# DallinClark/RealTimeRaytracer

Measured on AMD Instinct MI355X. Metric: Mrays/sec at 1920x1080 1spp (all rays: primary + shadow), higher is better.
Workload: dtype f32

## Files before the change

realtimeraytracer_amd/csrc/kernels/rtr_device.h:

```cpp
#pragma once
#include <hip/hip_runtime.h>
#include <stdint.h>
#include "../../../include/rtr_types.h"
#include "../../../include/rtr_math.h"

namespace rtrdev {

struct DeviceTexture { const uint8_t* pixels; uint32_t width, height, channels, _pad; };

constexpr uint32_t kLightTriRecord = 4;

struct DeviceScene {
    const uint4* nodes;
    const RtrBvhGrid* grid;
    const uint4* nodes4;
    uint32_t numNodes4;
    const float4* tris;
    const RtrVertex* vertices;
    const uint32_t* indices;
    const RtrObjectInfo* objects;
    const RtrAreaLightInfo* lights;
    const float4* lightTris;
    const uint32_t* lightTriFirst;
    const float* xforms;
// ... 376 lines not shown
__device__ __forceinline__ size_t out_index(const RenderArgs& ra, uint32_t px, uint32_t lrow, uint32_t gy) {
    return (size_t)(ra.directRows ? gy : lrow) * ra.width + px;
}

__device__ __forceinline__ rtr_v3 primary_dir(const RenderArgs& ra, uint32_t px, uint32_t py, uint32_t i) {
    const float jx = rtr_random(px + i), jy = rtr_random(px + i * 322u);
    const float offx = ((float)px + jx) - 0.5f, offy = ((float)py + jy) - 0.5f;
    const rtr_v3 pw = rtr_madd(rtr_madd(rtr_ld3(ra.cam.topLeftViewportCorner), rtr_ld3(ra.cam.horizontalViewportDelta), offx),
                               rtr_ld3(ra.cam.verticalViewportDelta), offy);
    return rtr_normalize(rtr_sub(pw, rtr_ld3(ra.cam.position)));
}

struct Accum { rtr_v3 analytic, shadowed, unshadowed, avgNormal, avgPosition; };

struct Surface {
    rtr_v3 hitPoint, hitNormal, viewDir, color, mDiffuse, mSpecular;
    float roughness, metallic, om;
    float4 t1, t2;
};

template <bool SHADE, bool STATS>
__device__ __forceinline__ bool fetch_surface(const DeviceScene& sc, const RenderArgs& ra, const HitRec& h, rtr_v3 rayDir,
                                              bool wantAnalytic, Accum& o, Surface& sf, LocalStats& st) {
    if (h.custom == RTR_MISS) {
        if (SHADE) {
            rtr_v3 sky = rtr_ld3(sc.skyLinear);
            if (sc.hdri.pixels) {
                const rtr_v3 dir = rtr_normalize(rayDir);
                const float hu = rtr_atan2(dir.z, dir.x) / (2.0f * 3.14159265f) + 0.5f;
                float hv = rtr_acos(rtr_clamp(dir.y, -1.0f, 1.0f)) / 3.14159265f;
                hv = 1.0f - hv;
                const float4 tx = sample_tex<STATS>(sc.hdri, hu, hv, st);
                sky = rtr_mk(rtr_to_linear(tx.x), rtr_to_linear(tx.y), rtr_to_linear(tx.z));
            }
            o.analytic = rtr_add(o.analytic, sky); o.unshadowed = rtr_add(o.unshadowed, sky); o.shadowed = rtr_add(o.shadowed, sky);
        }
        return false;
    }
    if (h.custom < sc.numLights) {
        if (SHADE) {
            const rtr_v3 lc = rtr_ld3(sc.lights[h.custom].color);
            o.analytic = rtr_add(o.analytic, lc); o.unshadowed = rtr_add(o.unshadowed, lc); o.shadowed = rtr_add(o.shadowed, lc);
        }
        return false;
    }
    const rtr_v3 camPos = rtr_ld3(ra.cam.position);
    if (STATS) st.hits++;
    const RtrObjectInfo* oi = sc.objects + (h.custom - sc.numLights);
    const uint32_t vOff = oi->vertexOffset, iOff = oi->indexOffset;
    const uint32_t i0 = sc.indices[3u * h.prim + 0u + iOff];
    const uint32_t i1 = sc.indices[3u * h.prim + 1u + iOff];
    const uint32_t i2 = sc.indices[3u * h.prim + 2u + iOff];
    const float4* va = reinterpret_cast<const float4*>(sc.vertices + (i0 + vOff));
    const float4* vb = reinterpret_cast<const float4*>(sc.vertices + (i1 + vOff));
    const float4* vc = reinterpret_cast<const float4*>(sc.vertices + (i2 + vOff));
    const rtr_v3 p0 = f4xyz(va[0]), p1 = f4xyz(vb[0]), p2 = f4xyz(vc[0]);
    const rtr_v3 n0 = f4xyz(va[1]), n1 = f4xyz(vb[1]), n2 = f4xyz(vc[1]);
    const float b0 = 1.0f - h.u - h.v, b1 = h.u, b2 = h.v;
    const rtr_v3 localPos = rtr_madd(rtr_madd(rtr_scale(p0, b0), p1, b1), p2, b2);
    const rtr_v3 hitPoint = rtr_xform_point34(sc.xforms + 12u * h.custom, localPos);
    const rtr_v3 nsum = rtr_madd(rtr_madd(rtr_scale(n0, b0), n1, b1), n2, b2);
    const float* nm = sc.nmats + 12u * h.custom;
    rtr_v3 hitNormal;
    if (rtr_dot(nsum, nsum) > 0.0f) {
        hitNormal = rtr_normalize(rtr_mul33(nm, rtr_normalize(nsum)));
    } else {
        const rtr_v3 g = rtr_cross(rtr_sub(p1, p0), rtr_sub(p2, p0));
        rtr_v3 n = rtr_normalize(rtr_mul33(nm, rtr_normalize(g)));
        if (rtr_dot(n, rayDir) > 0.0f) n = rtr_neg(n);
        hitNormal = n;
    }
    float metallic = oi->metallic;
    float rough = oi->specular;
    rtr_v3 color = rtr_mk(0, 0, 0);
    if (SHADE) {
        rtr_v3 col = rtr_ld3(oi->color);
        if (oi->usesColorMap | oi->usesSpecularMap | oi->usesMetallicMap) {
            const float4 ta = va[2], tb = vb[2], tc = vc[2];
            const float uu = rtr_fma(tc.x, b2, rtr_fma(tb.x, b1, ta.x * b0));
            const float vv = rtr_fma(tc.y, b2, rtr_fma(tb.y, b1, ta.y * b0));
            if (oi->usesColorMap != 0u) { const float4 t = sample_tex<STATS>(sc.textures[oi->colorIndex], uu, vv, st); col = rtr_mk(t.x, t.y, t.z); }
            if (oi->usesSpecularMap != 0u) rough = sample_tex<STATS>(sc.textures[oi->specularIndex], uu, vv, st).x;
            if (oi->usesMetallicMap != 0u) metallic = sample_tex<STATS>(sc.textures[oi->metallicIndex], uu, vv, st).x;
        }
        color = rtr_mk(rtr_to_linear(col.x), rtr_to_linear(col.y), rtr_to_linear(col.z));
    }
    const float roughness = 1.0f - rough;

    const rtr_v3 viewDir = rtr_normalize(rtr_sub(camPos, hitPoint));
    const float om = 1.0f - metallic;
    rtr_v3 mDiffuse = rtr_mk(0, 0, 0), mSpecular = rtr_mk(0, 0, 0);
    float4 t1 = make_float4(1, 0, 0, 1), t2 = make_float4(0, 0, 0, 0);
    if (SHADE) {
        o.avgNormal = rtr_add(o.avgNormal, hitNormal);
        o.avgPosition = rtr_add(o.avgPosition, hitPoint);
        mDiffuse = rtr_scale(color, om);
        mSpecular = rtr_mk(rtr_fma(color.x, metallic, 0.04f * om), rtr_fma(color.y, metallic, 0.04f * om),
                           rtr_fma(color.z, metallic, 0.04f * om));
        if (wantAnalytic) {
            const float dotNV = rtr_clamp(rtr_dot(hitNormal, viewDir), 0.0f, 1.0f);
            const float lu = rtr_fma(roughness, RTR_LUT_SCALE, RTR_LUT_BIAS);
            const float lv = rtr_fma(rtr_sqrt(1.0f - dotNV), RTR_LUT_SCALE, RTR_LUT_BIAS);
            t1 = sample_lut(sc.ltc1, lu, lv);
            t2 = sample_lut(sc.ltc2, lu, lv);
        }
    }
    sf.hitPoint = hitPoint; sf.hitNormal = hitNormal; sf.viewDir = viewDir; sf.color = color;
    sf.mDiffuse = mDiffuse; sf.mSpecular = mSpecular; sf.roughness = roughness; sf.metallic = metallic; sf.om = om;
    sf.t1 = t1; sf.t2 = t2;
    return true;
}

__device__ __forceinline__ rtr_v3 surface_diffuse(float om, rtr_v3 color) {
    return rtr_mk((om * color.x) / RTR_PI_F, (om * color.y) / RTR_PI_F, (om * color.z) / RTR_PI_F);
}
__device__ __forceinline__ rtr_v3 area_sample_contrib(rtr_v3 hitNormal, rtr_v3 viewDir, float roughness, rtr_v3 mSpecular, rtr_v3 currDiffuse,
                                                      rtr_v3 lcol, float lintensity, float pdf, rtr_v3 sampledLightDir, float lightDistance) {
    const rtr_v3 halfVector = rtr_normalize(rtr_add(viewDir, sampledLightDir));
    const float cosTheta = rtr_clamp(rtr_dot(viewDir, halfVector), 0.0f, 1.0f);
    const float Dg = GGX_Distribution(hitNormal, halfVector, roughness);
    const float G = GGX_PartialGeometryTerm(viewDir, hitNormal, halfVector, roughness) *
                    GGX_PartialGeometryTerm(sampledLightDir, hitNormal, halfVector, roughness);
    const rtr_v3 F = Fresnel_Schlick(cosTheta, mSpecular);
    const float NdotV = rtr_max(rtr_dot(hitNormal, viewDir), 0.1f);
    const float NdotL = rtr_max(rtr_dot(hitNormal, sampledLightDir), 0.1f);
    const float den = 4.0f * NdotV * NdotL;
    const rtr_v3 currSpecular = rtr_mk(((Dg * F.x) * G) / den, ((Dg * F.y) * G) / den, ((Dg * F.z) * G) / den);
    const float attenuation = 1.0f / (lightDistance * lightDistance);
    const rtr_v3 BRDF = rtr_add(currSpecular, currDiffuse);
    const rtr_v3 Lr = rtr_mk((((lcol.x * lintensity) * NdotL) * attenuation) * 10.0f, (((lcol.y * lintensity) * NdotL) * attenuation) * 10.0f,
                             (((lcol.z * lintensity) * NdotL) * attenuation) * 10.0f);
    return rtr_mk((BRDF.x * Lr.x) / pdf, (BRDF.y * Lr.y) / pdf, (BRDF.z * Lr.z) / pdf);
}
__device__ __forceinline__ rtr_v3 directional_light_dir() { return rtr_normalize(rtr_mk(-1.0f, 1.0f, -0.5f)); }
__device__ __forceinline__ rtr_v3 directional_contrib(rtr_v3 hitNormal, rtr_v3 viewDir, float roughness, rtr_v3 mSpecular, rtr_v3 currDiffuse) {
    const rtr_v3 directLightDir = directional_light_dir();
    const rtr_v3 directLightColor = rtr_mk(1.0f, 1.0f, 0.5f);
    const float directLightIntensity = 0.2f;
    const rtr_v3 halfVector = rtr_normalize(rtr_add(viewDir, directLightDir));
    const float cosTheta = rtr_clamp(rtr_dot(viewDir, halfVector), 0.0f, 1.0f);
    const float Dg = GGX_Distribution(hitNormal, halfVector, roughness);
    const float G = GGX_PartialGeometryTerm(viewDir, hitNormal, halfVector, roughness) *
                    GGX_PartialGeometryTerm(directLightDir, hitNormal, halfVector, roughness);
    const rtr_v3 F = Fresnel_Schlick(cosTheta, mSpecular);
    const float NdotV = rtr_max(rtr_dot(hitNormal, viewDir), 5.0f);
    const float NdotL = rtr_max(rtr_dot(hitNormal, directLightDir), 0.0001f);
    const float den = 4.0f * NdotV * NdotL;
    const rtr_v3 currSpecular = rtr_mk(((Dg * F.x) * G) / den, ((Dg * F.y) * G) / den, ((Dg * F.z) * G) / den);
    const rtr_v3 BRDF = rtr_add(currSpecular, currDiffuse);
    const rtr_v3 Lr = rtr_mk(((directLightColor.x * directLightIntensity) * NdotL) * 20.0f, ((directLightColor.y * directLightIntensity) * NdotL) * 20.0f,
                             ((directLightColor.z * directLightIntensity) * NdotL) * 20.0f);
    return rtr_mul(BRDF, Lr);
}
__device__ __forceinline__ rtr_v3 light_sample_pos(const rtr_v3* P, uint32_t s, uint32_t px, uint32_t py, uint32_t frame) {
    const uint32_t seed = s + px * 733u + py * 1933u + frame;
    float r1 = rtr_random(seed), r2 = rtr_random(seed + 100u);
    if (r1 + r2 > 1.0f) { r1 = 1.0f - r1; r2 = 1.0f - r2; }
    return rtr_madd(rtr_madd(P[0], rtr_sub(P[1], P[0]), r1), rtr_sub(P[2], P[0]), r2);
}

constexpr uint32_t kDirectionalSlot = 0xffffffffu;
#ifndef RTR_INTO_EXPR
#define RTR_INTO_EXPR (rtr_dot(hitNormal, lightVec) < 0.0f)
#endif
template <class Policy, bool STATS>
__device__ __forceinline__ void light_loops(const DeviceScene& sc, const RenderArgs& ra, uint32_t px, uint32_t py,
                                            const Surface& sf, uint32_t want, Accum& o, Policy& pol, LocalStats& st) {
    const bool wantAnalytic = (want & 1u) != 0u, wantUnshadowed = (want & 2u) != 0u;
    const rtr_v3 hitPoint = sf.hitPoint, hitNormal = sf.hitNormal, viewDir = sf.viewDir, color = sf.color;
    const rtr_v3 mDiffuse = sf.mDiffuse, mSpecular = sf.mSpecular;
    const float roughness = sf.roughness, om = sf.om;
    const float4 t1 = sf.t1, t2 = sf.t2;
    const rtr_v3 shadowOrigin = rtr_madd(hitPoint, hitNormal, 0.01f);
    const rtr_v3 currDiffuse = surface_diffuse(om, color);

    for (uint32_t li = 0; li < ra.info.numAreaLights; ++li) {
        const RtrAreaLightInfo* L = sc.lights + li;
        if (STATS) st.lightFetch++;
        const rtr_v3 lcol = rtr_ld3(L->color);
        const float lintensity = L->intensity;
        const uint32_t lnt = L->numTriangles;
        const bool twoSided = L->isTwoSided != 0u;
        for (uint32_t ti = 0; ti < lnt; ++ti) {
            if (STATS) st.lightTriFetch++;
            const float4* rec = sc.lightTris + (size_t)(sc.lightTriFirst[li] + ti) * kLightTriRecord;
            const float4 r0 = rec[0], r1 = rec[1], r2 = rec[2], r3 = rec[3];
            rtr_v3 P[3];
            P[0] = rtr_mk(r0.x, r0.y, r0.z); P[1] = rtr_mk(r1.x, r1.y, r1.z); P[2] = rtr_mk(r2.x, r2.y, r2.z);
            const float pdf = r1.w;
            const rtr_v3 lightNormal = rtr_mk(r3.x, r3.y, r3.z);
            if (!twoSided) {
                if (rtr_dot(lightNormal, rtr_sub(hitPoint, P[0])) < 0.0f) continue;
            }
            rtr_v3 shadowedSample = rtr_mk(0, 0, 0), unshadowedSample = rtr_mk(0, 0, 0);
            pol.slots_at((sc.lightTriFirst[li] + ti) * ra.numShadowRays);
            for (uint32_t s = 0; s < ra.numShadowRays; ++s) {
                const rtr_v3 lightSamplePos = light_sample_pos(P, s, px, py, ra.info.frame);
                const rtr_v3 lightVec = rtr_sub(lightSamplePos, hitPoint);
                const rtr_v3 sampledLightDir = rtr_normalize(lightVec);
                const float lightDistance = rtr_length(lightVec);
                const bool occ = pol.occluded(shadowOrigin, sampledLightDir, lightDistance - 0.5f, lightVec, RTR_INTO_EXPR);
                if (Policy::kShade && (wantUnshadowed || !occ)) {
                    const float currShadow = occ ? 0.0f : 1.0f;
                    const rtr_v3 contrib = area_sample_contrib(hitNormal, viewDir, roughness, mSpecular, currDiffuse, lcol, lintensity, pdf, sampledLightDir, lightDistance);
                    shadowedSample = rtr_madd(shadowedSample, contrib, currShadow);
                    unshadowedSample = rtr_add(unshadowedSample, contrib);
                }
            }
            if (Policy::kShade) {
                const float ns = (float)ra.numShadowRays;
                shadowedSample = rtr_mk(shadowedSample.x / ns, shadowedSample.y / ns, shadowedSample.z / ns);
                unshadowedSample = rtr_mk(unshadowedSample.x / ns, unshadowedSample.y / ns, unshadowedSample.z / ns);
                if (wantAnalytic) {
                    const float diffuse = LTC_Evaluate(hitNormal, viewDir, hitPoint, true, t1, P, lightNormal, twoSided, sc.ltc2);
                    const float spec = LTC_Evaluate(hitNormal, viewDir, hitPoint, false, t1, P, lightNormal, twoSided, sc.ltc2);
                    const rtr_v3 fres = rtr_mk(rtr_fma(1.0f - mSpecular.x, t2.y, mSpecular.x * t2.x),
                                               rtr_fma(1.0f - mSpecular.y, t2.y, mSpecular.y * t2.x),
                                               rtr_fma(1.0f - mSpecular.z, t2.y, mSpecular.z * t2.x));
                    o.analytic = rtr_add(o.analytic, rtr_mk(((lcol.x * lintensity) * rtr_fma(mDiffuse.x, diffuse, spec * fres.x)) * 5.0f,
                                                            ((lcol.y * lintensity) * rtr_fma(mDiffuse.y, diffuse, spec * fres.y)) * 5.0f,
                                                            ((lcol.z * lintensity) * rtr_fma(mDiffuse.z, diffuse, spec * fres.z)) * 5.0f));
                }
                o.shadowed = rtr_add(o.shadowed, shadowedSample);
                o.unshadowed = rtr_add(o.unshadowed, unshadowedSample);
            }
        }
    }
    const rtr_v3 directLightDir = directional_light_dir();
    if (rtr_dot(hitNormal, directLightDir) <= 0.0f) return;
    pol.slots_at(kDirectionalSlot);
    const bool occ = pol.occluded(shadowOrigin, directLightDir, 10000.0f, directLightDir, false);
    if (Policy::kShade && (wantUnshadowed || wantAnalytic || !occ)) {
        const float currShadow = occ ? 0.0f : 1.0f;
        const rtr_v3 contrib = directional_contrib(hitNormal, viewDir, roughness, mSpecular, currDiffuse);
        o.shadowed = rtr_madd(o.shadowed, contrib, currShadow);
        o.unshadowed = rtr_add(o.unshadowed, contrib);
        o.analytic = rtr_add(o.analytic, contrib);
    }
}

__device__ __forceinline__ void light_tri_record(const RtrAreaLightInfo* L, const RtrVertex* vertices, const uint32_t* indices,
                                                 uint32_t ti, float4* rec) {
    const uint32_t lvOff = L->vertexOffset, liOff = L->indexOffset;
    const uint32_t j0 = indices[ti * 3u + 0u + liOff];
    const uint32_t j1 = indices[ti * 3u + 1u + liOff];
    const uint32_t j2 = indices[ti * 3u + 2u + liOff];
    rtr_v3 P[3];
    P[0] = rtr_xform_point44cm(L->transform, rtr_ld3(vertices[j0 + lvOff].position));
    P[1] = rtr_xform_point44cm(L->transform, rtr_ld3(vertices[j1 + lvOff].position));
    P[2] = rtr_xform_point44cm(L->transform, rtr_ld3(vertices[j2 + lvOff].position));
    rtr_v3 lightNormal = rtr_cross(rtr_sub(P[2], P[1]), rtr_sub(P[0], P[1]));
    const float area = rtr_length(lightNormal) * 0.5f;
    const float pdf = 1.0f / (area * 0.7f);
    lightNormal = rtr_normalize(lightNormal);
    rec[0] = make_float4(P[0].x, P[0].y, P[0].z, area);
    rec[1] = make_float4(P[1].x, P[1].y, P[1].z, pdf);
    rec[2] = make_float4(P[2].x, P[2].y, P[2].z, 0.f);
    rec[3] = make_float4(lightNormal.x, lightNormal.y, lightNormal.z, 0.f);
}

template <class Policy, bool STATS>
__device__ __forceinline__ void shade_sample(const DeviceScene& sc, const RenderArgs& ra, uint32_t px, uint32_t py,
                                             const HitRec& h, rtr_v3 rayDir, uint32_t want, Accum& o,
                                             Policy& pol, LocalStats& st) {
    Surface sf;
    if (!fetch_surface<Policy::kShade, STATS>(sc, ra, h, rayDir, (want & 1u) != 0u, o, sf, st)) return;
    light_loops<Policy, STATS>(sc, ra, px, py, sf, want, o, pol, st);
}

__device__ __forceinline__ uint32_t tonemap_pack(rtr_v3 c) {
    return rtr_pack_bgra8(rtr_to_srgb(rtr_aces(c.x)), rtr_to_srgb(rtr_aces(c.y)), rtr_to_srgb(rtr_aces(c.z)));
}

struct FrameOut {
    uint32_t* img[8];
    float4* hdr;
};

constexpr uint32_t kMaxBatch = 32;
struct FrameBatch {
    RenderArgs ra[kMaxBatch];
    FrameOut   fo[kMaxBatch];
    uint32_t   n;
};
static_assert(sizeof(FrameBatch) + sizeof(DeviceScene) + 256 <= 16384, "a launch passes DeviceScene + FrameBatch + a few pointers by value");
__device__ __forceinline__ uint32_t batch_frame(uint32_t g, uint32_t planeStride, uint32_t& q) {
    const uint32_t b = (uint32_t)__builtin_amdgcn_readfirstlane((int)(g / planeStride));
    q = g - b * planeStride;
    return b;
}

__device__ __forceinline__ void write_pixel(const RenderArgs& ra, const FrameOut& fo, size_t p, Accum o) {
    const float n = (float)ra.spp;
    rtr_v3 sh = rtr_mk(o.shadowed.x / n, o.shadowed.y / n, o.shadowed.z / n);
    const rtr_v3 un = rtr_mk(o.unshadowed.x / n, o.unshadowed.y / n, o.unshadowed.z / n);
    const rtr_v3 an = rtr_mk(o.analytic.x / n, o.analytic.y / n, o.analytic.z / n);
    if (fo.hdr) {
        if (ra.accumulate) {
            float4 h = fo.hdr[p];
            h.x += sh.x; h.y += sh.y; h.z += sh.z; h.w += 1.0f;
            fo.hdr[p] = h;
            const float inv = (float)(ra.accumulatedFrames + 1u);
            sh = rtr_mk(h.x / inv, h.y / inv, h.z / inv);
        } else {
            fo.hdr[p] = make_float4(sh.x, sh.y, sh.z, 1.0f);
        }
    }
    if (fo.img[1]) fo.img[1][p] = tonemap_pack(sh);
    if (fo.img[2]) fo.img[2][p] = tonemap_pack(un);
    if (fo.img[0]) fo.img[0][p] = tonemap_pack(an);
    if (fo.img[6]) {
        const rtr_v3 a = rtr_normalize(rtr_mk(o.avgNormal.x / n, o.avgNormal.y / n, o.avgNormal.z / n));
        fo.img[6][p] = rtr_pack_bgra8(a.x, a.y, a.z);
    }
    if (fo.img[7]) fo.img[7][p] = rtr_pack_bgra8(o.avgPosition.x / n, o.avgPosition.y / n, o.avgPosition.z / n);
}

__device__ __forceinline__ void write_pixel_framebuffer(const RenderArgs& ra, const FrameOut& fo, size_t p, rtr_v3 shadowed) {
    const float n = (float)ra.spp;
    rtr_v3 sh = rtr_mk(shadowed.x / n, shadowed.y / n, shadowed.z / n);
    if (fo.hdr) {
        if (ra.accumulate) {
            float4 h = fo.hdr[p];
            h.x += sh.x; h.y += sh.y; h.z += sh.z; h.w += 1.0f;
            fo.hdr[p] = h;
            const float inv = (float)(ra.accumulatedFrames + 1u);
            sh = rtr_mk(h.x / inv, h.y / inv, h.z / inv);
        } else {
            fo.hdr[p] = make_float4(sh.x, sh.y, sh.z, 1.0f);
        }
    }
    if (fo.img[1]) fo.img[1][p] = tonemap_pack(sh);
}

}
```

realtimeraytracer_amd/csrc/kernels/rtr_kernels.hip:

```cpp
#include "rtr_kernels.h"

#include <algorithm>
#include <cstdlib>
#include <cstring>

namespace rtrdev {

constexpr int kBlock = 256;

template <bool STATS, int STACK>
struct InlinePolicy {
    static constexpr bool kShade = true;
    __device__ __forceinline__ void slots_at(uint32_t) {}
    const DeviceScene& sc; int32_t* stack; LocalStats& st;
    __device__ __forceinline__ bool occluded(rtr_v3 o, rtr_v3 d, float tmax, rtr_v3, bool) {
        HitRec h;
        return trace<true, STATS, kBlock>(sc, stack, o, d, 0.001f, tmax, h, st);
    }
};

__device__ __forceinline__ uint32_t wave_sum_u32(uint32_t v) {
#pragma unroll
    for (int o = 32; o > 0; o >>= 1) v += __shfl_xor(v, o);
    return v;
// ... 163 lines not shown
    HitRec h;
    if (STATS) trace<false, true, kPrimBlock, 16, 8>(sc, stack, camPos, dir, 0.001f, 10000.0f, h, st);
    else {
        const uint32_t oct = ray_octant(sc, camPos, dir);
        const uint32_t woct = (uint32_t)__builtin_amdgcn_readfirstlane((int)oct);
        switch (__ballot(oct != woct) != 0ull ? 8u : woct) {
            case 0: trace<false, false, kPrimBlock, 16, 0>(sc, stack, camPos, dir, 0.001f, 10000.0f, h, st); break;
            case 1: trace<false, false, kPrimBlock, 16, 1>(sc, stack, camPos, dir, 0.001f, 10000.0f, h, st); break;
            case 2: trace<false, false, kPrimBlock, 16, 2>(sc, stack, camPos, dir, 0.001f, 10000.0f, h, st); break;
            case 3: trace<false, false, kPrimBlock, 16, 3>(sc, stack, camPos, dir, 0.001f, 10000.0f, h, st); break;
            case 4: trace<false, false, kPrimBlock, 16, 4>(sc, stack, camPos, dir, 0.001f, 10000.0f, h, st); break;
            case 5: trace<false, false, kPrimBlock, 16, 5>(sc, stack, camPos, dir, 0.001f, 10000.0f, h, st); break;
            case 6: trace<false, false, kPrimBlock, 16, 6>(sc, stack, camPos, dir, 0.001f, 10000.0f, h, st); break;
            case 7: trace<false, false, kPrimBlock, 16, 7>(sc, stack, camPos, dir, 0.001f, 10000.0f, h, st); break;
            default: trace<false, false, kPrimBlock, 16, 8>(sc, stack, camPos, dir, 0.001f, 10000.0f, h, st); break;
        }
    }
    const size_t k = (size_t)plane * planeBlocks * kPrimBlock + q;
    if (h.custom == RTR_STACK_OVERFLOW) redoList[atomicAdd(redoCount, 1u)] = (uint32_t)k;
    else {
        hitTuvp[k] = make_float4(h.t, h.u, h.v, __uint_as_float(h.prim));
        hitCustom[k] = h.custom;
        origin_leaf_store(rayOrigin, k, h.leaf);
    }
    if (STATS) st.flush(stats);
}

template <bool STATS>
__global__ __launch_bounds__(kBlock) void k_primary_packet(DeviceScene sc, FrameBatch fb, float4* hitTuvp, uint32_t* hitCustom, float4* rayOrigin, Counters* stats, uint32_t planeBlocks) {
    __shared__ uint4 s_stack[kBlock / 64][64];
    const uint32_t wave = threadIdx.x >> 6, lane = threadIdx.x & 63u;
    const uint32_t plane = blockIdx.x / planeBlocks;
    const RenderArgs& ra = fb.ra[plane / fb.ra[0].spp];
    const uint32_t i = plane % fb.ra[0].spp;
    const uint32_t q = (blockIdx.x - plane * planeBlocks) * kBlock + threadIdx.x;
    uint32_t px = 0, lrow = 0, py = 0;
    const bool valid = pixel_of(ra, q, px, lrow, py);
    unsigned long long active = __ballot(valid);
    if (active == 0ull) return;
    LocalStats st;
    const rtr_v3 o = rtr_ld3(ra.cam.position);
    const rtr_v3 d = valid ? primary_dir(ra, px, py, i) : rtr_mk(0.f, 0.f, 1.f);
    const float tmin = 0.001f, tmax = 10000.0f;
    if (STATS && valid) { st.rays++; st.primary++; }
    const rtr_v3 idir = rtr_mk(rtr_safe_rcp_dir(d.x), rtr_safe_rcp_dir(d.y), rtr_safe_rcp_dir(d.z));
    rtr_v3 ga, gb;
    rtr_ray_grid(o, idir, sc.grid->origin, sc.grid->scale, &ga, &gb);
    HitRec best; best.t = tmax; best.u = 0.f; best.v = 0.f; best.custom = RTR_MISS; best.prim = RTR_MISS; best.leaf = 0;
    const uint4* __restrict__ nodes = sc.nodes;
    const float4* __restrict__ tris = sc.tris;
    uint32_t sp = 0;
    int32_t cur = 0;
    for (;;) {
        const bool mine = ((active >> lane) & 1ull) != 0ull;
        bool pop = true;
        if (cur >= 0) {
            const uint4 a = nodes[2 * cur], b = nodes[2 * cur + 1];
            if (STATS && mine) st.nodes++;
            float tl = 0.f, tr = 0.f;
            const bool hl = mine && slab_pair(a.x, a.y, b.x, ga, gb, tmin, best.t, tl);
            const bool hr = mine && slab_pair(a.z, a.w, b.y, ga, gb, tmin, best.t, tr);
            const unsigned long long mL = __ballot(hl), mR = __ballot(hr);
            if ((mL | mR) != 0ull) {
                pop = false;
                if (mR == 0ull) { cur = (int32_t)b.z; active = mL; }
                else if (mL == 0ull) { cur = (int32_t)b.w; active = mR; }
                else {
                    const uint32_t rNear = (uint32_t)__popcll(__ballot(hl && hr && tr < tl)), lNear = (uint32_t)__popcll(__ballot(hl && hr && !(tr < tl)));
                    const bool rFirst = rNear > lNear;
                    if (lane == 0u) {
                        const unsigned long long m2 = rFirst ? mL : mR;
                        s_stack[wave][sp] = make_uint4(rFirst ? b.z : b.w, (uint32_t)m2, (uint32_t)(m2 >> 32), 0u);
                    }
                    ++sp;
                    cur = (int32_t)(rFirst ? b.w : b.z); active = rFirst ? mR : mL;
                }
            }
        } else {
            const uint32_t code = (uint32_t)~cur;
            const uint32_t first = code >> 3, cnt = (code & 7u) + 1u;
            for (uint32_t k = 0; k < cnt; ++k) {
                const float4 q0 = tris[3u * (first + k)], q1 = tris[3u * (first + k) + 1u], q2 = tris[3u * (first + k) + 2u];
                if (mine) {
                    if (STATS) st.tris++;
                    float t, u, v;
                    if (rtr_mt_intersect(o, d, f4xyz(q0), f4xyz(q1), f4xyz(q2), tmin, &t, &u, &v) && t < tmax) {
                        const uint32_t cu = __float_as_uint(q0.w), pr = __float_as_uint(q1.w);
                        if (!(__float_as_uint(q2.w) & 1u) || alpha_pass<STATS>(sc, cu, pr, u, v, st)) {
                            if (t < best.t || (t == best.t && (cu < best.custom || (cu == best.custom && pr < best.prim)))) {
                                best.t = t; best.u = u; best.v = v; best.custom = cu; best.prim = pr; best.leaf = cur;
                            }
                        }
                    }
                }
            }
        }
        if (pop) {
            if (sp == 0u) break;
            --sp;
            const uint4 e = s_stack[wave][sp];
            cur = __builtin_amdgcn_readfirstlane((int32_t)e.x);
            active = (unsigned long long)(uint32_t)__builtin_amdgcn_readfirstlane((int)e.y) | ((unsigned long long)(uint32_t)__builtin_amdgcn_readfirstlane((int)e.z) << 32);
        }
    }
    if (valid) {
        const size_t k = (size_t)plane * planeBlocks * kBlock + q;
        hitTuvp[k] = make_float4(best.t, best.u, best.v, __uint_as_float(best.prim));
        hitCustom[k] = best.custom;
        origin_leaf_store(rayOrigin, k, best.leaf);
    }
    if (STATS) st.flush(stats);
}

template <bool STATS>
__global__ __launch_bounds__(kBlock) void k_primary_tail(DeviceScene sc, FrameBatch fb, float4* hitTuvp, uint32_t* hitCustom, float4* rayOrigin,
                                                         const uint32_t* __restrict__ redoCount, const uint32_t* __restrict__ redoList,
                                                         int32_t* __restrict__ spill, uint32_t planeStride, Counters* stats) {
    const uint32_t n = *redoCount;
    if (n == 0) return;
    int32_t* stack = spill + blockIdx.x * kBlock + threadIdx.x;
    LocalStats st;
    for (uint32_t j = blockIdx.x * kBlock + threadIdx.x; j < n; j += gridDim.x * kBlock) {
        const uint32_t k = redoList[j];
        const uint32_t plane = k / planeStride, q = k % planeStride;
        const RenderArgs& ra = fb.ra[plane / fb.ra[0].spp];
        const uint32_t i = plane % fb.ra[0].spp;
        uint32_t px, lrow, py;
        if (!pixel_of(ra, q, px, lrow, py)) continue;
        HitRec h;
        trace<false, STATS, 64 * kBlock>(sc, stack, rtr_ld3(ra.cam.position), primary_dir(ra, px, py, i), 0.001f, 10000.0f, h, st);
        if (STATS) { st.rays--; st.primary--; }
        hitTuvp[k] = make_float4(h.t, h.u, h.v, __uint_as_float(h.prim));
        hitCustom[k] = h.custom;
        origin_leaf_store(rayOrigin, k, h.leaf);
    }
    if (STATS) st.flush(stats);
}

__device__ __forceinline__ uint32_t wave_sum(uint32_t v) {
#pragma unroll
    for (int o = 32; o > 0; o >>= 1) v += __shfl_xor(v, o);
    return v;
}
__device__ __forceinline__ uint32_t wave_total(uint32_t v) {
    v += (uint32_t)__builtin_amdgcn_update_dpp(0, (int)v, 0xB1, 0xf, 0xf, false);
    v += (uint32_t)__builtin_amdgcn_update_dpp(0, (int)v, 0x4E, 0xf, 0xf, false);
    v += (uint32_t)__builtin_amdgcn_update_dpp(0, (int)v, 0x141, 0xf, 0xf, false);
    v += (uint32_t)__builtin_amdgcn_update_dpp(0, (int)v, 0x140, 0xf, 0xf, false);
    v += (uint32_t)__builtin_amdgcn_update_dpp(0, (int)v, 0x142, 0xa, 0xf, false);
    v += (uint32_t)__builtin_amdgcn_update_dpp(0, (int)v, 0x143, 0xc, 0xf, false);
    return (uint32_t)__builtin_amdgcn_readlane((int)v, 63);
}

constexpr uint32_t kGenBlock = 1024;
__global__ __launch_bounds__(kGenBlock) void k_shadow_gen(DeviceScene sc, FrameBatch fb, const float4* hitTuvp,
                                                          const uint32_t* hitCustom, RayQueue queue, uint32_t* count, uint32_t planeStride) {
    __shared__ uint32_t s_off[kGenBlock / 64], s_tot[kGenBlock / 64], s_base;
    uint32_t q;
    const uint32_t frame = batch_frame(blockIdx.x * kGenBlock + threadIdx.x, planeStride, q);
    const RenderArgs& ra = fb.ra[frame < fb.n ? frame : 0u];
    const size_t plane0 = (size_t)frame * ra.spp;
    const uint32_t wave = threadIdx.x >> 6;
    uint32_t px = 0, lrow = 0, py = 0;
    const bool live = frame < fb.n && pixel_of(ra, q, px, lrow, py);
    LocalStats st;
    Accum acc = zero_accum();
    const bool single = ra.spp == 1u;
    Surface sf0;
    bool surf0 = false;
    uint32_t n = 0;
    if (live) {
        CountPolicy cp{0};
        for (uint32_t i = 0; i < ra.spp; ++i) {
            const size_t k = (plane0 + i) * planeStride + q;
            const float4 r = hitTuvp[k];
            HitRec h; h.t = r.x; h.u = r.y; h.v = r.z; h.prim = __float_as_uint(r.w); h.custom = hitCustom[k];
            Surface sf;
            const bool surf = fetch_surface<false, false>(sc, ra, h, primary_dir(ra, px, py, i), false, acc, sf, st);
            if (surf) light_loops<CountPolicy, false>(sc, ra, px, py, sf, 0u, acc, cp, st);
            if (i == 0) { sf0 = sf; surf0 = surf; }
        }
        n = cp.n;
    }
    const uint32_t total = wave_sum(n);
    if ((threadIdx.x & 63u) == 0) { s_tot[wave] = total; s_off[wave] = 0; }
    __syncthreads();
    if (threadIdx.x == 0) {
        uint32_t t = 0;
        for (uint32_t w = 0; w < kGenBlock / 64; ++w) t += s_tot[w];
        s_base = t ? atomicAdd(count, t) : 0u;
    }
    __syncthreads();
    uint32_t base = s_base;
    for (uint32_t w = 0; w < wave; ++w) base += s_tot[w];
    if (!live || n == 0) return;
    for (uint32_t i = 0; i < ra.spp; ++i) {
        const size_t k = (plane0 + i) * planeStride + q;
        EmitPolicy pol{queue, (EmitPolicy::lds_word)&s_off[wave], base, (uint32_t)k};
        if (single) {
            if (surf0) { queue_store_origin(queue, k, sf0.hitPoint, sf0.hitNormal); light_loops<EmitPolicy, false>(sc, ra, px, py, sf0, 0u, acc, pol, st); }
        } else {
            const float4 r = hitTuvp[k];
            HitRec h; h.t = r.x; h.u = r.y; h.v = r.z; h.prim = __float_as_uint(r.w); h.custom = hitCustom[k];
            Surface sf;
            if (fetch_surface<false, false>(sc, ra, h, primary_dir(ra, px, py, i), false, acc, sf, st)) {
                queue_store_origin(queue, k, sf.hitPoint, sf.hitNormal);
                light_loops<EmitPolicy, false>(sc, ra, px, py, sf, 0u, acc, pol, st);
            }
        }
    }
}

constexpr size_t kBinnedMinRays = (size_t)10 << 20;
constexpr uint32_t kBinnedMinNodes = 1u << 16;
#ifndef RTR_GEN_OCT_BLOCK
#define RTR_GEN_OCT_BLOCK 512
#endif
constexpr uint32_t kGenOctBlock = RTR_GEN_OCT_BLOCK;
#ifndef RTR_GEN_OCT_WAVES
#define RTR_GEN_OCT_WAVES 7
#endif
#if RTR_GEN_OCT_WAVES > 0
#define RTR_GEN_OCT_ATTR __attribute__((amdgpu_waves_per_eu(RTR_GEN_OCT_WAVES, 8)))
#else
#define RTR_GEN_OCT_ATTR
#endif
__global__ __launch_bounds__(kGenOctBlock) RTR_GEN_OCT_ATTR void k_shadow_gen_oct(DeviceScene sc, FrameBatch fb, const float4* hitTuvp, const uint32_t* hitCustom,
                                                              RayQueue queue, uint32_t* ctrl, uint32_t planeStride, uint2* lists,
                                                              uint32_t listStride, uint32_t kBatch, uint32_t nt) {
    constexpr uint32_t kWaves = kGenOctBlock / 64;
    __shared__ uint32_t s_tot[kWaves][8], s_run[kWaves][8];
    uint32_t q;
    const uint32_t frame = batch_frame(blockIdx.x * kGenOctBlock + threadIdx.x, planeStride, q);
    const RenderArgs& ra = fb.ra[frame < fb.n ? frame : 0u];
    const size_t plane0 = (size_t)frame * ra.spp;
    const uint32_t wave = threadIdx.x >> 6;
    uint32_t px = 0, lrow = 0, py = 0;
    const bool live = frame < fb.n && pixel_of(ra, q, px, lrow, py);
    LocalStats st;
    Accum acc = zero_accum();
    const bool single = ra.spp == 1u;
    Surface sf0;
    bool surf0 = false;
    CountOctPolicy cp{0ull, 0ull};
    if (live) {
        for (uint32_t i = 0; i < ra.spp; ++i) {
            const size_t k = (plane0 + i) * planeStride + q;
            const float4 r = hitTuvp[k];
            HitRec h; h.t = r.x; h.u = r.y; h.v = r.z; h.prim = __float_as_uint(r.w); h.custom = hitCustom[k];
            Surface sf;
            bool surf = fetch_surface<false, false>(sc, ra, h, primary_dir(ra, px, py, i), false, acc, sf, st);
#if RTR_EXP_DOUBLE_FETCH_GEN
            if (surf) {
                HitRec h2 = h; h2.u = h.u + sf.hitPoint.x * (float)(ra.spp - 1u) * 1.0e-30f; h2.v = h.v + sf.hitNormal.y * (float)(ra.spp - 1u) * 1.0e-30f;
                h2.prim = h.prim + (__float_as_uint(sf.hitPoint.z) == 0x7fc12345u ? 1u : 0u);
                Surface sf2;
                if (fetch_surface<false, false>(sc, ra, h2, primary_dir(ra, px, py, i), false, acc, sf2, st)) sf = sf2;
            }
#endif
            if (surf) light_loops<CountOctPolicy, false>(sc, ra, px, py, sf, 0u, acc, cp, st);
            if (i == 0) { sf0 = sf; surf0 = surf; }
        }
    }
    uint32_t mine = 0;
#pragma unroll
    for (uint32_t o = 0; o < 8; ++o) {
        const uint32_t c = (uint32_t)(((o < 4 ? cp.lo : cp.hi) >> ((o & 3u) * 16u)) & 0xffffull);
        mine += c;
        const uint32_t t = wave_total(c);
        if ((threadIdx.x & 63u) == 0) s_tot[wave][o] = t;
    }
    __syncthreads();
    if (threadIdx.x < kQueueLists) {
        const uint32_t o = threadIdx.x / kQueueRegions, x = threadIdx.x % kQueueRegions;
        uint32_t before = 0, len = 0, total = 0;
#pragma unroll
        for (uint32_t oo = 0; oo < 8; ++oo) {
            uint32_t t = 0;
#pragma unroll
            for (uint32_t w = 0; w < kWaves; ++w) t += s_tot[w][oo];
            before += oo < o ? t : 0u;
            len = oo == o ? t : len;
            total += t;
        }
        const uint32_t kB = (kBatch >= 512u && blockIdx.x * 8u >= gridDim.x * 7u) ? kBatch / 2u : kBatch;
        const uint32_t nb = (len + kB - 1) / kB;
        const uint32_t b0 = (x + kQueueRegions - blockIdx.x % kQueueRegions) % kQueueRegions;
        const uint32_t cnt = b0 < nb ? (nb - b0 + kQueueRegions - 1) / kQueueRegions : 0u;
        uint32_t at = 0, pos = 0;
        if (threadIdx.x == 0 && total) at = atomicAdd(ctrl, total);
        if (cnt) pos = atomicAdd(ctrl + kQueueListLens + threadIdx.x, cnt);
        const uint32_t first = (uint32_t)__builtin_amdgcn_readfirstlane((int)at) + before;
        if (x == 0) {
            uint32_t c = first;
            for (uint32_t w = 0; w < kWaves; ++w) { s_run[w][o] = c; c += s_tot[w][o]; }
        }
        for (uint32_t j = 0; j < cnt; ++j) {
            const uint32_t f = (b0 + j * kQueueRegions) * kB;
            lists[(size_t)threadIdx.x * listStride + pos + j] = make_uint2(first + f, len - f < kB ? len - f : kB);
        }
    }
    __syncthreads();
    if (!live || mine == 0) return;
    for (uint32_t i = 0; i < ra.spp; ++i) {
        const size_t k = (plane0 + i) * planeStride + q;
        EmitOctPolicy pol{queue, (EmitOctPolicy::lds_word)&s_run[wave][0], (uint32_t)k, nt};
        if (single) {
            if (surf0) { queue_store_origin(queue, k, sf0.hitPoint, sf0.hitNormal); light_loops<EmitOctPolicy, false>(sc, ra, px, py, sf0, 0u, acc, pol, st); }
        } else {
            const float4 r = hitTuvp[k];
            HitRec h; h.t = r.x; h.u = r.y; h.v = r.z; h.prim = __float_as_uint(r.w); h.custom = hitCustom[k];
            Surface sf;
            if (fetch_surface<false, false>(sc, ra, h, primary_dir(ra, px, py, i), false, acc, sf, st)) {
                queue_store_origin(queue, k, sf.hitPoint, sf.hitNormal);
                light_loops<EmitOctPolicy, false>(sc, ra, px, py, sf, 0u, acc, pol, st);
            }
        }
    }
}

#ifndef RTR_REFILL_LDS
#define RTR_REFILL_LDS 1
#endif
#ifndef RTR_LIST_SHARE
#define RTR_LIST_SHARE 1
#endif
constexpr int kTailBlocks = 64;
constexpr int32_t kDone = (int32_t)0x80000000;
constexpr int32_t kAbandoned = (int32_t)0x80000001;
constexpr uint32_t kBatchDefault = 256, kBatchLong = 512;
constexpr size_t kBatchLongQueue = (size_t)100 << 20;

constexpr uint32_t kResNone = 3u;
#ifndef RTR_TRACE_BLOCK
#define RTR_TRACE_BLOCK 256
#endif
constexpr int kTraceBlock = RTR_TRACE_BLOCK;
#ifndef RTR_TRI_AUX
#define RTR_TRI_AUX 0
#endif
#ifndef RTR_NODE_AUX
#define RTR_NODE_AUX 0
#endif
#ifndef RTR_SHADOW_STACK
#define RTR_SHADOW_STACK RTR_WIDE_STACK
#endif
#ifndef RTR_TRACE_TOP
#define RTR_TRACE_TOP 40
#endif
constexpr uint32_t kTopNodes = (uint32_t)RTR_TRACE_TOP * (RTR_TRACE_BLOCK / 256);

template <int STACK>
__global__ __launch_bounds__(kBlock) void k_shadow_trace(DeviceScene sc, const RayQueue queue,
                                                              const uint32_t* __restrict__ count, uint32_t* nextBatch,
                                                              uint8_t* __restrict__ vis, uint32_t visFill, uint32_t kBatch, uint32_t kRefill,
                                                              uint32_t kInnerMin, uint32_t* overflow, uint32_t overflowCap) {
    __shared__ int32_t s_stack[(STACK + 1) * kBlock];
    int32_t* lds = s_stack + threadIdx.x;
    lds[0] = kDone;
    const uint32_t n = *count;
    uint32_t batchPos = 0, batchEnd = 0;
    bool exhausted = false;
    const uint32_t regionLen = ((n + kQueueRegions - 1) / kQueueRegions + kBatch - 1) / kBatch * kBatch;
    const uint32_t myRegion = blockIdx.x % kQueueRegions;
    uint32_t regionTry = 0;
    int32_t cur = kDone;
    int sp = 0;
    rtr_v3 o = rtr_mk(0, 0, 0), d = rtr_mk(0, 0, 0), ga = rtr_mk(0, 0, 0), gb = rtr_mk(0, 0, 0);
    float tmax = 0.f;
    uint32_t slot = 0, rayIndex = 0, res = kResNone, occ = 0;
    const float tmin = 0.001f;
    typedef uint32_t u32x4 __attribute__((ext_vector_type(4)));
    const __amdgpu_buffer_rsrc_t nodeBuf = __builtin_amdgcn_make_buffer_rsrc((void*)sc.nodes, 0, 0xffffffff, 0x00020000);
    const __amdgpu_buffer_rsrc_t triBuf = __builtin_amdgcn_make_buffer_rsrc((void*)sc.tris, 0, 0xffffffff, 0x00020000);

    for (;;) {
        const unsigned long long idle = __ballot(cur == kDone);
        const uint32_t nIdle = (uint32_t)__popcll(idle);
        if (nIdle >= kRefill || nIdle == 64u) {
            if (cur == kDone && res != kResNone) {
                if (res == 2u) { const uint32_t at = atomicAdd(overflow, 1u); if (at < overflowCap) overflow[1u + at] = rayIndex; }
                else { if (res != visFill) vis[slot] = (uint8_t)res; occ += res; }
                res = kResNone;
            }
            if (!exhausted) {
                if (batchPos == batchEnd) {
                    for (;;) {
                        if (regionTry >= kQueueRegions) { exhausted = true; break; }
                        const uint32_t r = (myRegion + regionTry) % kQueueRegions;
                        const uint32_t lo = r * regionLen;
                        uint32_t hi = lo + regionLen; if (hi > n) hi = n;
                        uint32_t b = hi;
                        if (lo < hi) {
                            uint32_t got = 0;
                            if ((threadIdx.x & 63u) == 0) got = atomicAdd(nextBatch + 16u * r, kBatch);
                            got = (uint32_t)__builtin_amdgcn_readfirstlane((int)got);
                            b = got < regionLen ? lo + got : hi;
                        }
                        if (b < hi) { batchPos = b; batchEnd = (b + kBatch < hi) ? b + kBatch : hi; break; }
                        ++regionTry;
                    }
                }
                if (!exhausted) {
                    const uint32_t avail = batchEnd - batchPos;
                    const uint32_t prefix = __builtin_amdgcn_mbcnt_hi((uint32_t)(idle >> 32), __builtin_amdgcn_mbcnt_lo((uint32_t)idle, 0u));
                    if (cur == kDone && prefix < avail) {
                        rayIndex = batchPos + prefix;
                        queue_load(queue, rayIndex, o, d, tmax, slot, 0u);
                        if (!(tmax > tmin)) {
                            if (visFill != 0u) vis[slot] = 0;
                        } else {
                            const rtr_v3 idir = rtr_mk(rtr_safe_rcp_dir(d.x), rtr_safe_rcp_dir(d.y), rtr_safe_rcp_dir(d.z));
                            rtr_ray_grid(o, idir, sc.grid->origin, sc.grid->scale, &ga, &gb);
                            cur = 0; sp = 0; res = 0u;
                        }
                    }
                    batchPos += (nIdle < avail) ? nIdle : avail;
                }
            }
        }
        if (__ballot(cur != kDone) == 0ull) {
            if (exhausted) break;
            continue;
        }
        for (;;) {
            const unsigned long long innerMask = __ballot(cur >= 0);
            if (innerMask == 0ull) break;
            if ((uint32_t)__popcll(innerMask) <= kInnerMin && __ballot(cur < 0 && cur != kDone) != 0ull) break;
            if (cur >= 0) {
                const int32_t nodeOff = cur << 5;
                const u32x4 a = __builtin_amdgcn_raw_buffer_load_b128(nodeBuf, nodeOff, 0, 0);
                const u32x4 b = __builtin_amdgcn_raw_buffer_load_b128(nodeBuf, nodeOff + 16, 0, 0);
                const int32_t top = lds[sp * kBlock];
                float tl, tr;
                const bool hl = slab_pair(a.x, a.y, b.x, ga, gb, tmin, tmax, tl);
                const bool hr = slab_pair(a.z, a.w, b.y, ga, gb, tmin, tmax, tr);
                const bool swap = tr < tl;
                const int32_t c0 = (int32_t)b.z, c1 = (int32_t)b.w;
                const bool both = hl && hr, none = !(hl || hr);
                const bool second = both ? swap : !hl;
                int32_t next = second ? c1 : c0;
                const bool push = both && sp < STACK;
                if (push) { ++sp; lds[sp * kBlock] = swap ? c0 : c1; }
                if (both && !push) { res = 2u; next = kDone; }
                if (none) { next = top; --sp; }
                cur = next;
            }
        }
        if (cur < 0 && cur != kDone) {
            const uint32_t code = (uint32_t)~cur;
            const uint32_t first = code >> 3, cnt = (code & 7u) + 1u;
            bool hit = false;
            for (uint32_t i = 0; i < cnt && !hit; ++i) {
                const int32_t triOff = (int32_t)((first + i) * 48u);
                const u32x4 r0 = __builtin_amdgcn_raw_buffer_load_b128(triBuf, triOff, 0, 0);
                const u32x4 r1 = __builtin_amdgcn_raw_buffer_load_b128(triBuf, triOff + 16, 0, 0);
                const u32x4 r2 = __builtin_amdgcn_raw_buffer_load_b128(triBuf, triOff + 32, 0, 0);
                const float4 q0 = make_float4(__uint_as_float(r0.x), __uint_as_float(r0.y), __uint_as_float(r0.z), __uint_as_float(r0.w));
                const float4 q1 = make_float4(__uint_as_float(r1.x), __uint_as_float(r1.y), __uint_as_float(r1.z), __uint_as_float(r1.w));
                const float4 q2 = make_float4(__uint_as_float(r2.x), __uint_as_float(r2.y), __uint_as_float(r2.z), __uint_as_float(r2.w));
                float t, u, v;
                if (rtr_mt_intersect(o, d, f4xyz(q0), f4xyz(q1), f4xyz(q2), tmin, &t, &u, &v) && t < tmax) {
                    hit = true;
                    if (__float_as_uint(q2.w) & 1u) {
                        LocalStats st;
                        hit = alpha_pass<false>(sc, __float_as_uint(q0.w), __float_as_uint(q1.w), u, v, st);
                    }
                }
// ... 1112 lines not shown
```

Before: 16490.

## Park shadow sample pairs and hit surface in LDS across count/emit passes

Shadow-ray generation kernels now precompute each pixel's light-sample random pairs once into LDS columns when the shadow-ray count is small, reusing them in both the counting and emitting passes. The octant generator also parks the single-spp hit point and normal in LDS instead of keeping a full Surface live in registers across the block barrier, and reduces per-wave totals in grouped register batches. The intent is to cut recomputation of RNG and lower register pressure so more waves fit. In exchange it uses a large LDS allocation per block, which may itself limit occupancy, and it drops the live/surface check before the emit loop, relying on mine==0 for pixels with no hit.

```diff
diff --git a/realtimeraytracer_amd/csrc/kernels/rtr_device.h b/realtimeraytracer_amd/csrc/kernels/rtr_device.h
--- a/realtimeraytracer_amd/csrc/kernels/rtr_device.h
+++ b/realtimeraytracer_amd/csrc/kernels/rtr_device.h
@@ -552,20 +552,31 @@
                              ((directLightColor.z * directLightIntensity) * NdotL) * 20.0f);
     return rtr_mul(BRDF, Lr);
 }
-__device__ __forceinline__ rtr_v3 light_sample_pos(const rtr_v3* P, uint32_t s, uint32_t px, uint32_t py, uint32_t frame) {
-    const uint32_t seed = s + px * 733u + py * 1933u + frame;
+struct SamplePair { float r1, r2; };
+__device__ __forceinline__ uint32_t light_sample_seed0(uint32_t px, uint32_t py, uint32_t frame) { return px * 733u + py * 1933u + frame; }
+__device__ __forceinline__ SamplePair light_sample_pair(uint32_t seed) {
     float r1 = rtr_random(seed), r2 = rtr_random(seed + 100u);
     if (r1 + r2 > 1.0f) { r1 = 1.0f - r1; r2 = 1.0f - r2; }
-    return rtr_madd(rtr_madd(P[0], rtr_sub(P[1], P[0]), r1), rtr_sub(P[2], P[0]), r2);
-}
+    return SamplePair{r1, r2};
+}
+__device__ __forceinline__ rtr_v3 light_sample_at(const rtr_v3* P, SamplePair r) {
+    return rtr_madd(rtr_madd(P[0], rtr_sub(P[1], P[0]), r.r1), rtr_sub(P[2], P[0]), r.r2);
+}
+__device__ __forceinline__ rtr_v3 light_sample_pos(const rtr_v3* P, uint32_t s, uint32_t px, uint32_t py, uint32_t frame) {
+    return light_sample_at(P, light_sample_pair(s + light_sample_seed0(px, py, frame)));
+}
+struct DrawnSamples {
+    uint32_t px, py, frame;
+    __device__ __forceinline__ SamplePair pair(uint32_t s) const { return light_sample_pair(s + light_sample_seed0(px, py, frame)); }
+};
 
 constexpr uint32_t kDirectionalSlot = 0xffffffffu;
 #ifndef RTR_INTO_EXPR
 #define RTR_INTO_EXPR (rtr_dot(hitNormal, lightVec) < 0.0f)
 #endif
-template <class Policy, bool STATS>
-__device__ __forceinline__ void light_loops(const DeviceScene& sc, const RenderArgs& ra, uint32_t px, uint32_t py,
-                                            const Surface& sf, uint32_t want, Accum& o, Policy& pol, LocalStats& st) {
+template <class Policy, bool STATS, class Samples>
+__device__ __forceinline__ void light_loops_from(const DeviceScene& sc, const RenderArgs& ra, const Samples& smp,
+                                                 const Surface& sf, uint32_t want, Accum& o, Policy& pol, LocalStats& st) {
     const bool wantAnalytic = (want & 1u) != 0u, wantUnshadowed = (want & 2u) != 0u;
     const rtr_v3 hitPoint = sf.hitPoint, hitNormal = sf.hitNormal, viewDir = sf.viewDir, color = sf.color;
     const rtr_v3 mDiffuse = sf.mDiffuse, mSpecular = sf.mSpecular;
@@ -595,7 +606,7 @@
             rtr_v3 shadowedSample = rtr_mk(0, 0, 0), unshadowedSample = rtr_mk(0, 0, 0);
             pol.slots_at((sc.lightTriFirst[li] + ti) * ra.numShadowRays);
             for (uint32_t s = 0; s < ra.numShadowRays; ++s) {
-                const rtr_v3 lightSamplePos = light_sample_pos(P, s, px, py, ra.info.frame);
+                const rtr_v3 lightSamplePos = light_sample_at(P, smp.pair(s));
                 const rtr_v3 lightVec = rtr_sub(lightSamplePos, hitPoint);
                 const rtr_v3 sampledLightDir = rtr_normalize(lightVec);
                 const float lightDistance = rtr_length(lightVec);
@@ -638,6 +649,11 @@
         o.analytic = rtr_add(o.analytic, contrib);
     }
 }
+template <class Policy, bool STATS>
+__device__ __forceinline__ void light_loops(const DeviceScene& sc, const RenderArgs& ra, uint32_t px, uint32_t py,
+                                            const Surface& sf, uint32_t want, Accum& o, Policy& pol, LocalStats& st) {
+    light_loops_from<Policy, STATS>(sc, ra, DrawnSamples{px, py, ra.info.frame}, sf, want, o, pol, st);
+}
 
 __device__ __forceinline__ void light_tri_record(const RtrAreaLightInfo* L, const RtrVertex* vertices, const uint32_t* indices,
                                                  uint32_t ti, float4* rec) {
diff --git a/realtimeraytracer_amd/csrc/kernels/rtr_kernels.hip b/realtimeraytracer_amd/csrc/kernels/rtr_kernels.hip
--- a/realtimeraytracer_amd/csrc/kernels/rtr_kernels.hip
+++ b/realtimeraytracer_amd/csrc/kernels/rtr_kernels.hip
@@ -339,10 +339,31 @@
     return (uint32_t)__builtin_amdgcn_readlane((int)v, 63);
 }
 
+constexpr uint32_t kParkedPairs = 4;
+typedef __attribute__((address_space(3))) uint32_t* lds_column;
+template <uint32_t BLOCK>
+struct ParkedSamples {
+    lds_column pairs;
+    uint32_t seed0;
+    bool parked;
+    __device__ __forceinline__ void draw(uint32_t ns) const {
+        if (!parked) return;
+        for (uint32_t s = 0; s < ns; ++s) {
+            const SamplePair r = light_sample_pair(s + seed0);
+            pairs[2u * s * BLOCK] = __float_as_uint(r.r1); pairs[(2u * s + 1u) * BLOCK] = __float_as_uint(r.r2);
+        }
+    }
+    __device__ __forceinline__ SamplePair pair(uint32_t s) const {
+        if (parked) return SamplePair{__uint_as_float(pairs[2u * s * BLOCK]), __uint_as_float(pairs[(2u * s + 1u) * BLOCK])};
+        return light_sample_pair(s + seed0);
+    }
+};
+
 constexpr uint32_t kGenBlock = 1024;
 __global__ __launch_bounds__(kGenBlock) void k_shadow_gen(DeviceScene sc, FrameBatch fb, const float4* hitTuvp,
                                                           const uint32_t* hitCustom, RayQueue queue, uint32_t* count, uint32_t planeStride) {
     __shared__ uint32_t s_off[kGenBlock / 64], s_tot[kGenBlock / 64], s_base;
+    __shared__ uint32_t s_pairs[2u * kParkedPairs * kGenBlock];
     uint32_t q;
     const uint32_t frame = batch_frame(blockIdx.x * kGenBlock + threadIdx.x, planeStride, q);
     const RenderArgs& ra = fb.ra[frame < fb.n ? frame : 0u];
@@ -356,15 +377,17 @@
     Surface sf0;
     bool surf0 = false;
     uint32_t n = 0;
+    const ParkedSamples<kGenBlock> smp{(lds_column)&s_pairs[threadIdx.x], light_sample_seed0(px, py, ra.info.frame), ra.numShadowRays <= kParkedPairs};
     if (live) {
         CountPolicy cp{0};
+        smp.draw(ra.numShadowRays);
         for (uint32_t i = 0; i < ra.spp; ++i) {
             const size_t k = (plane0 + i) * planeStride + q;
             const float4 r = hitTuvp[k];
             HitRec h; h.t = r.x; h.u = r.y; h.v = r.z; h.prim = __float_as_uint(r.w); h.custom = hitCustom[k];
             Surface sf;
             const bool surf = fetch_surface<false, false>(sc, ra, h, primary_dir(ra, px, py, i), false, acc, sf, st);
-            if (surf) light_loops<CountPolicy, false>(sc, ra, px, py, sf, 0u, acc, cp, st);
+            if (surf) light_loops_from<CountPolicy, false>(sc, ra, smp, sf, 0u, acc, cp, st);
             if (i == 0) { sf0 = sf; surf0 = surf; }
         }
         n = cp.n;
@@ -385,14 +408,14 @@
         const size_t k = (plane0 + i) * planeStride + q;
         EmitPolicy pol{queue, (EmitPolicy::lds_word)&s_off[wave], base, (uint32_t)k};
         if (single) {
-            if (surf0) { queue_store_origin(queue, k, sf0.hitPoint, sf0.hitNormal); light_loops<EmitPolicy, false>(sc, ra, px, py, sf0, 0u, acc, pol, st); }
+            if (surf0) { queue_store_origin(queue, k, sf0.hitPoint, sf0.hitNormal); light_loops_from<EmitPolicy, false>(sc, ra, smp, sf0, 0u, acc, pol, st); }
         } else {
             const float4 r = hitTuvp[k];
             HitRec h; h.t = r.x; h.u = r.y; h.v = r.z; h.prim = __float_as_uint(r.w); h.custom = hitCustom[k];
             Surface sf;
             if (fetch_surface<false, false>(sc, ra, h, primary_dir(ra, px, py, i), false, acc, sf, st)) {
                 queue_store_origin(queue, k, sf.hitPoint, sf.hitNormal);
-                light_loops<EmitPolicy, false>(sc, ra, px, py, sf, 0u, acc, pol, st);
+                light_loops_from<EmitPolicy, false>(sc, ra, smp, sf, 0u, acc, pol, st);
             }
         }
     }
@@ -404,6 +427,7 @@
 #define RTR_GEN_OCT_BLOCK 512
 #endif
 constexpr uint32_t kGenOctBlock = RTR_GEN_OCT_BLOCK;
+constexpr uint32_t kParkSurface = 6, kParkWords = kParkSurface + 2u * kParkedPairs;
 #ifndef RTR_GEN_OCT_WAVES
 #define RTR_GEN_OCT_WAVES 7
 #endif
@@ -417,6 +441,7 @@
                                                               uint32_t listStride, uint32_t kBatch, uint32_t nt) {
     constexpr uint32_t kWaves = kGenOctBlock / 64;
     __shared__ uint32_t s_tot[kWaves][8], s_run[kWaves][8];
+    __shared__ uint32_t s_park[kParkWords * kGenOctBlock];
     uint32_t q;
     const uint32_t frame = batch_frame(blockIdx.x * kGenOctBlock + threadIdx.x, planeStride, q);
     const RenderArgs& ra = fb.ra[frame < fb.n ? frame : 0u];
@@ -427,10 +452,11 @@
     LocalStats st;
     Accum acc = zero_accum();
     const bool single = ra.spp == 1u;
-    Surface sf0;
-    bool surf0 = false;
+    const lds_column park = (lds_column)&s_park[threadIdx.x];
+    const ParkedSamples<kGenOctBlock> smp{park + kParkSurface * kGenOctBlock, light_sample_seed0(px, py, ra.info.frame), ra.numShadowRays <= kParkedPairs};
     CountOctPolicy cp{0ull, 0ull};
     if (live) {
+        smp.draw(ra.numShadowRays);
         for (uint32_t i = 0; i < ra.spp; ++i) {
             const size_t k = (plane0 + i) * planeStride + q;
             const float4 r = hitTuvp[k];
@@ -445,8 +471,13 @@
                 if (fetch_surface<false, false>(sc, ra, h2, primary_dir(ra, px, py, i), false, acc, sf2, st)) sf = sf2;
             }
 #endif
-            if (surf) light_loops<CountOctPolicy, false>(sc, ra, px, py, sf, 0u, acc, cp, st);
-            if (i == 0) { sf0 = sf; surf0 = surf; }
+            if (surf) {
+                if (single) {
+                    park[0u * kGenOctBlock] = __float_as_uint(sf.hitPoint.x); park[1u * kGenOctBlock] = __float_as_uint(sf.hitPoint.y); park[2u * kGenOctBlock] = __float_as_uint(sf.hitPoint.z);
+                    park[3u * kGenOctBlock] = __float_as_uint(sf.hitNormal.x); park[4u * kGenOctBlock] = __float_as_uint(sf.hitNormal.y); park[5u * kGenOctBlock] = __float_as_uint(sf.hitNormal.z);
+                }
+                light_loops_from<CountOctPolicy, false>(sc, ra, smp, sf, 0u, acc, cp, st);
+            }
         }
     }
     uint32_t mine = 0;
@@ -461,14 +492,21 @@
     if (threadIdx.x < kQueueLists) {
         const uint32_t o = threadIdx.x / kQueueRegions, x = threadIdx.x % kQueueRegions;
         uint32_t before = 0, len = 0, total = 0;
+        uint32_t tot[8] = {0u, 0u, 0u, 0u, 0u, 0u, 0u, 0u};
+#pragma unroll
+        for (uint32_t w0 = 0; w0 < kWaves; w0 += 4u) {
+#pragma unroll
+            for (uint32_t w = w0; w < w0 + 4u && w < kWaves; ++w) {
+#pragma unroll
+                for (uint32_t oo = 0; oo < 8; ++oo) tot[oo] += s_tot[w][oo];
+            }
+            asm volatile("" : "+v"(tot[0]), "+v"(tot[1]), "+v"(tot[2]), "+v"(tot[3]), "+v"(tot[4]), "+v"(tot[5]), "+v"(tot[6]), "+v"(tot[7]) : : "memory");
+        }
 #pragma unroll
         for (uint32_t oo = 0; oo < 8; ++oo) {
-            uint32_t t = 0;
-#pragma unroll
-            for (uint32_t w = 0; w < kWaves; ++w) t += s_tot[w][oo];
-            before += oo < o ? t : 0u;
-            len = oo == o ? t : len;
-            total += t;
+            before += oo < o ? tot[oo] : 0u;
+            len = oo == o ? tot[oo] : len;
+            total += tot[oo];
         }
         const uint32_t kB = (kBatch >= 512u && blockIdx.x * 8u >= gridDim.x * 7u) ? kBatch / 2u : kBatch;
         const uint32_t nb = (len + kB - 1) / kB;
@@ -488,19 +526,23 @@
         }
     }
     __syncthreads();
-    if (!live || mine == 0) return;
+    if (mine == 0) return;
     for (uint32_t i = 0; i < ra.spp; ++i) {
         const size_t k = (plane0 + i) * planeStride + q;
         EmitOctPolicy pol{queue, (EmitOctPolicy::lds_word)&s_run[wave][0], (uint32_t)k, nt};
         if (single) {
-            if (surf0) { queue_store_origin(queue, k, sf0.hitPoint, sf0.hitNormal); light_loops<EmitOctPolicy, false>(sc, ra, px, py, sf0, 0u, acc, pol, st); }
+            Surface sf0 = {};
+            sf0.hitPoint = rtr_mk(__uint_as_float(park[0u * kGenOctBlock]), __uint_as_float(park[1u * kGenOctBlock]), __uint_as_float(park[2u * kGenOctBlock]));
+            sf0.hitNormal = rtr_mk(__uint_as_float(park[3u * kGenOctBlock]), __uint_as_float(park[4u * kGenOctBlock]), __uint_as_float(park[5u * kGenOctBlock]));
+            queue_store_origin(queue, k, sf0.hitPoint, sf0.hitNormal);
+            light_loops_from<EmitOctPolicy, false>(sc, ra, smp, sf0, 0u, acc, pol, st);
         } else {
             const float4 r = hitTuvp[k];
             HitRec h; h.t = r.x; h.u = r.y; h.v = r.z; h.prim = __float_as_uint(r.w); h.custom = hitCustom[k];
             Surface sf;
             if (fetch_surface<false, false>(sc, ra, h, primary_dir(ra, px, py, i), false, acc, sf, st)) {
                 queue_store_origin(queue, k, sf.hitPoint, sf.hitNormal);
-                light_loops<EmitOctPolicy, false>(sc, ra, px, py, sf, 0u, acc, pol, st);
+                light_loops_from<EmitOctPolicy, false>(sc, ra, smp, sf, 0u, acc, pol, st);
             }
         }
     }
```

After: 16650, median of 6. +1.0%, better.
